# ajpowelsnl/mhm2_proxy

Hardware: AMD Instinct MI355X
Metric: k-mers/s (whole node), k=21 150bp reads (higher is better)
Workload: dtype u64

## Files before the change

mhm2_proxy_amd/csrc/kcount_kernels.hip:

```cpp
#include <hip/hip_runtime.h>
#include <type_traits>

#include <algorithm>

#include "kcount_launch.hpp"
#include "kmer_ops.hpp"

namespace mhm {

template <int NL>
constexpr int kTile() {
  return TILE_BASES[NL];
}
template <int NL>
constexpr int kEThreads() {
  return E_THREADS_NL[NL];
}
template <int NL>
constexpr int kPTile() {
  return P_TILE[NL];
}
template <int NL>
constexpr int kPThreads() {
  return P_THREADS[NL];
// ... 1357 lines not shown
    for (int i = threadIdx.x; i < SKETCH_FH; i += NT)
      if (fh[i]) atomicAdd(&fhist[i], fh[i]);
  for (int i = threadIdx.x; i < SKETCH_M; i += NT)
    if (reg[i]) {
      atomicMax(&hll[i], reg[i]);
      if (!(blockIdx.x & 1u)) atomicMax(&hll[SKETCH_M + 1 + i], reg[i]);
    }
  if (threadIdx.x == 0 && s_ext) atomicAdd(&hll[SKETCH_M], s_ext);
}

__global__ void k_init_fine(const unsigned long long *coarse_base, const unsigned long long *coarse_fcap, uint32_t n_coarse,
                            int fine_bits, unsigned long long *base, unsigned long long *cursor) {
  const uint64_t i = (uint64_t)blockIdx.x * blockDim.x + threadIdx.x;
  if (i >= ((uint64_t)n_coarse << fine_bits)) return;
  const uint64_t c = i >> fine_bits, d = i & ((1ull << fine_bits) - 1);
  const unsigned long long b = coarse_base[c] + d * coarse_fcap[c];
  base[i] = b;
  cursor[i] = b;
}

__global__ __launch_bounds__(256) void k_count_windows(ReadsView rv, int k, unsigned long long *out, unsigned int *err) {
  __shared__ unsigned long long s_acc[4];
  unsigned long long acc = 0;
  bool bad = false;
  const uint64_t stride = (uint64_t)gridDim.x * blockDim.x;
  for (uint64_t r0 = (uint64_t)blockIdx.x * blockDim.x + threadIdx.x; r0 < rv.n_reads; r0 += 4 * stride) {
    uint64_t a[4], b[4];
#pragma unroll
    for (int u = 0; u < 4; u++) {
      const uint64_t r = r0 + u * stride, rr = r < rv.n_reads ? r : rv.n_reads - 1;
      a[u] = rv.offs[rr];
      b[u] = rv.offs[rr + 1];
    }
#pragma unroll
    for (int u = 0; u < 4; u++) {
      if (r0 + u * stride >= rv.n_reads) break;
      bad |= b[u] < a[u] || b[u] - a[u] > 65535;
      const uint64_t L = b[u] - a[u];
      acc += (b[u] >= a[u] && L > (uint64_t)k + 1) ? L - k - 1 : 0;
    }
  }
  if (blockIdx.x == 0 && threadIdx.x == 0)
    bad |= rv.offs[0] != rv.obase + rv.head || rv.offs[rv.n_reads] - rv.obase != rv.n_bases;
  if (bad) atomicOr(err, 4u);
  acc = wave_sum_u64(acc);
  if ((threadIdx.x & 63) == 0) s_acc[threadIdx.x >> 6] = acc;
  __syncthreads();
  if (threadIdx.x == 0) {
    const unsigned long long t = s_acc[0] + s_acc[1] + s_acc[2] + s_acc[3];
    if (t) atomicAdd(out, t);
  }
}

__global__ __launch_bounds__(256) void k_expand_nibbles(const uint8_t *nib, uint8_t *arena, uint64_t b0, uint64_t n) {
  const uint64_t a0 = b0 & ~15ull, end = b0 + n;
  const uint64_t p0 = a0 + ((uint64_t)blockIdx.x * blockDim.x + threadIdx.x) * 16;
  if (p0 >= end) return;
  uint32_t w[4] = {0, 0, 0, 0};
#pragma unroll
  for (int i = 0; i < 16; i++) {
    const uint64_t p = p0 + i;
    if (p >= b0 && p < end) {
      const uint64_t j = p - b0;
      const uint32_t v = (nib[j >> 1] >> (4 * (uint32_t)(j & 1))) & 15u;
      w[i >> 2] |= ((v & 7u) | ((v >> 3) * 0xf8u)) << (8 * (i & 3));
    }
  }
  if (p0 >= b0 && p0 + 16 <= end) {
    *(uint4 *)(arena + p0) = make_uint4(w[0], w[1], w[2], w[3]);
    return;
  }
#pragma unroll
  for (int i = 0; i < 16; i++) {
    const uint64_t p = p0 + i;
    if (p >= b0 && p < end) arena[p] = (uint8_t)(w[i >> 2] >> (8 * (i & 3)));
  }
}

__global__ __launch_bounds__(256) void k_offs_from_deltas(const uint32_t *d, uint64_t *offs, uint64_t n, uint64_t b0) {
  for (uint64_t i = (uint64_t)blockIdx.x * 256 + threadIdx.x; i < n; i += (uint64_t)gridDim.x * 256) offs[i] = b0 + d[i];
}

__global__ __launch_bounds__(1024) void k_scan(const unsigned long long *in, unsigned long long *base,
                                               unsigned long long *cursor, uint32_t n) {
  __shared__ unsigned long long wsum[17];
  const int tid = threadIdx.x, lane = tid & 63, wid = tid >> 6;
  const uint32_t per = (n + 1023) / 1024;
  const uint32_t lo = min((uint32_t)tid * per, n), hi = min(lo + per, n);
  unsigned long long s = 0;
  for (uint32_t i = lo; i < hi; i++) s += (in[i] + 3) & ~3ull;
  unsigned long long x = s;
#pragma unroll
  for (int d = 1; d < 64; d <<= 1) {
    unsigned long long y = __shfl_up(x, d, 64);
    if (lane >= d) x += y;
  }
  if (lane == 63) wsum[wid] = x;
  __syncthreads();
  if (tid == 0) {
    unsigned long long acc = 0;
    for (int w = 0; w < 16; w++) {
      unsigned long long t = wsum[w];
      wsum[w] = acc;
      acc += t;
    }
  }
  __syncthreads();
  unsigned long long run = wsum[wid] + x - s;
  for (uint32_t i = lo; i < hi; i++) {
    base[i] = run;
    cursor[i] = run;
    run += (in[i] + 3) & ~3ull;
  }
}


template <int NL>
constexpr int count_rpt() {
  return NL == 1 ? 4 : 1;
}

template <int NL>
__device__ __forceinline__ uint32_t slot_hash(const uint64_t *key) {
  if (NL == 1) {
    const uint32_t x = (uint32_t)(key[0] >> 32) * 0x9E3779B1u + (uint32_t)key[0] * 0x85EBCA77u;
    return x ^ (x >> 15);
  }
  uint64_t h = key[0] * 0x9E3779B97F4A7C15ull;
#pragma unroll
  for (int w = 1; w < NL; w++) h = (h ^ (h >> 31) ^ key[w]) * 0xC2B2AE3D27D4EB4Full;
  h ^= h >> 29;
  return (uint32_t)(h >> 32);
}

__device__ __forceinline__ int cmp_group(uint32_t key, int kshl, uint32_t ng) {
  return (int)(__umul24((key << kshl) >> 16, ng) >> 16);
}

template <typename K>
struct CountLds {
  K *keys;
  uint32_t *cnt;
  uint32_t *ext;
  int cap;
};

typedef __attribute__((address_space(3))) unsigned int lds_u32_t;
__device__ __forceinline__ uint32_t lds_add_late(unsigned int *p, uint32_t v) {
  lds_u32_t *q = (lds_u32_t *)p;
  asm volatile("" : "+v"(q));
  return __hip_atomic_fetch_add(q, v, __ATOMIC_RELAXED, __HIP_MEMORY_SCOPE_WORKGROUP);
}

constexpr int C_PROBE = 64;
template <int NL>
constexpr int count_batch() {
  return NL == 2 ? 1 : 2;
}
constexpr int GS_SLOTS = 4;

template <int GS>
__device__ __forceinline__ void read_group(const uint64_t *last, int g, uint64_t (&v)[GS]) {
  const ulonglong2 *q = (const ulonglong2 *)(last + GS * g);
  const ulonglong2 a = q[0];
  v[0] = a.x, v[1] = a.y;
  if constexpr (GS == 4) {
    const ulonglong2 b = q[1];
    v[2] = b.x, v[3] = b.y;
  }
}
template <int GS>
__device__ __forceinline__ void read_group(const uint32_t *last, int g, uint32_t (&v)[GS]) {
  if constexpr (GS == 4) {
    const uint4 a = *(const uint4 *)(last + 4 * g);
    v[0] = a.x, v[1] = a.y, v[2] = a.z, v[3] = a.w;
  } else {
    const uint2 a = *(const uint2 *)(last + 2 * g);
    v[0] = a.x, v[1] = a.y;
  }
}

template <int NL, typename K>
__device__ __forceinline__ bool rest_equal(const CountLds<K> &t, int slot, const uint64_t *key) {
  bool eq = true;
#pragma unroll
  for (int w = 0; w < NL - 1; w++) eq &= (t.keys[w * t.cap + slot] == key[w]);
  return eq;
}

constexpr int G_FULL = -8, G_BUSY = -9;
template <int NL, int GS, typename K>
__device__ __forceinline__ int examine_group(const CountLds<K> &t, const uint64_t *key, int g, const K (&v)[GS]) {
  const K kl = (K)key[NL - 1];
  if constexpr (NL == 1) {
    int r = G_FULL;
#pragma unroll
    for (int i = GS - 1; i >= 0; i--) r = v[i] == (K)KEY_EMPTY ? -1 - i : r;
#pragma unroll
    for (int i = GS - 1; i >= 0; i--) r = v[i] == kl ? GS * g + i : r;
    return r;
  }
  if constexpr (NL >= 2) {
    int r = G_FULL;
#pragma unroll
    for (int i = GS - 1; i >= 0; i--) r = v[i] == (K)KEY_EMPTY ? -1 - i : r;
#pragma unroll
    for (int i = GS - 1; i >= 0; i--) r = v[i] == (K)KEY_BUSY ? G_BUSY : r;
#pragma unroll
    for (int i = GS - 1; i >= 0; i--) r = v[i] == kl ? GS * g + i : r;
    if (r < 0 || rest_equal<NL>(t, r, key)) return r;
  }
  int found = -1, empty = -1;
  bool busy = false;
#pragma unroll
  for (int i = 0; i < GS; i++) {
    if (found < 0 && v[i] == kl && (NL == 1 || rest_equal<NL>(t, GS * g + i, key))) found = i;
    if (v[i] == (K)KEY_EMPTY && empty < 0) empty = i;
    if (NL > 1 && v[i] == (K)KEY_BUSY) busy = true;
  }
  if (found >= 0) return GS * g + found;
  if (busy) return G_BUSY;
  return empty >= 0 ? -1 - empty : G_FULL;
}

template <int NL, int GS, typename K>
__device__ int lds_insert(const CountLds<K> &t, const uint64_t *key, int g, int r) {
  K *last = t.keys + (NL - 1) * t.cap;
  const int ng = t.cap / GS;
  const K kl = (K)key[NL - 1];
  int probed = 0;
  for (int iter = 0; iter < (1 << 20); iter++) {
    if (r >= 0) return r;
    if (r == G_FULL) {
      if (++probed == C_PROBE * 4 / GS) return -1;
      g = (g + 1 == ng) ? 0 : g + 1;
    } else if (r != G_BUSY) {
      const int sl = GS * g + (-1 - r);
      const K want = (NL == 1) ? kl : (K)KEY_BUSY;
      K old;
      if constexpr (sizeof(K) == 4)
        old = atomicCAS((unsigned int *)&last[sl], 0xffffffffu, (unsigned int)want);
      else
        old = atomicCAS((unsigned long long *)&last[sl], (unsigned long long)KEY_EMPTY, (unsigned long long)want);
      if (old == (K)KEY_EMPTY) {
        if (NL > 1) {
#pragma unroll
          for (int w = 0; w < NL - 1; w++) t.keys[w * t.cap + sl] = (K)key[w];
          __hip_atomic_store(&last[sl], kl, __ATOMIC_RELEASE, __HIP_MEMORY_SCOPE_WORKGROUP);
        }
        return sl;
      }
      if (NL == 1 && old == kl) return sl;
    }
    K v[GS];
    read_group<GS>(last, g, v);
    r = examine_group<NL, GS>(t, key, g, v);
  }
  return -2;
}

template <int NL, int GS, typename K>
__device__ __forceinline__ int claim_home(const CountLds<K> &t, const uint64_t *key, int g, int r) {
  K *last = t.keys + (NL - 1) * t.cap;
  const int sl = GS * g + (-1 - r);
  const K kl = (K)key[NL - 1];
  if constexpr (NL == 1) {
    K old;
    if constexpr (sizeof(K) == 4)
      old = atomicCAS((unsigned int *)&last[sl], 0xffffffffu, (unsigned int)kl);
    else
      old = atomicCAS((unsigned long long *)&last[sl], (unsigned long long)KEY_EMPTY, (unsigned long long)kl);
    return (old == (K)KEY_EMPTY || old == kl) ? sl : r;
  } else {
    const K old = atomicCAS((unsigned long long *)&last[sl], (unsigned long long)KEY_EMPTY, (unsigned long long)KEY_BUSY);
    if (old != (K)KEY_EMPTY) return r;
#pragma unroll
    for (int w = 0; w < NL - 1; w++) t.keys[w * t.cap + sl] = (K)key[w];
    __hip_atomic_store(&last[sl], kl, __ATOMIC_RELEASE, __HIP_MEMORY_SCOPE_WORKGROUP);
    return sl;
  }
}

template <typename K>
__device__ __forceinline__ uint32_t lds_add(const CountLds<K> &t, int slot, uint32_t e) {
  const uint32_t old = atomicAdd(&t.cnt[slot], 1u);
  const int l = (int)((e >> 3) & 7u), r = (int)(e & 7u);
  if (l < 4) atomicAdd(&t.ext[(l >> 1) * t.cap + slot], (l & 1) ? 0x10000u : 1u);
  if (r < 4) atomicAdd(&t.ext[(2 + (r >> 1)) * t.cap + slot], (r & 1) ? 0x10000u : 1u);
  return old;
}

template <typename K>
__device__ __forceinline__ void lds_add_nr(const CountLds<K> &t, int slot, uint32_t e, uint32_t *dummy) {
  const uint32_t l = (e >> 3) & 7u, r = e & 7u;
  uint32_t *lw = l < 4u ? &t.ext[(l >> 1) * t.cap + slot] : &t.cnt[slot];
  atomicAdd(lw, (l & 1u) ? 0x10000u : 1u);
  uint32_t *rw = r < 4u ? &t.ext[(2 + (r >> 1)) * t.cap + slot] : dummy;
  atomicAdd(rw, (r & 1u) ? 0x10000u : 1u);
}

template <typename K>
__device__ __forceinline__ uint32_t slot_count(const CountLds<K> &t, int slot, bool cold) {
  const uint32_t c = t.cnt[slot];
  if (!cold) return c;
  if (c >> 31) return c & 0x7fffffffu;
  const uint32_t e0 = t.ext[slot], e1 = t.ext[t.cap + slot];
  return c + (e0 & 0xffffu) + (e0 >> 16) + (e1 & 0xffffu) + (e1 >> 16);
}

__device__ __forceinline__ void ext_clamp(uint32_t *p, int half) {
  uint32_t cur = __hip_atomic_load(p, __ATOMIC_RELAXED, __HIP_MEMORY_SCOPE_WORKGROUP);
  for (int iter = 0; iter < 4096; iter++) {
    const uint32_t f = half ? (cur >> 16) : (cur & 0xffffu);
    if (f < 0xC000u) break;
    const uint32_t nw = half ? ((cur & 0xffffu) | 0x80000000u) : ((cur & 0xffff0000u) | 0x8000u);
    const uint32_t prev = atomicCAS(p, cur, nw);
    if (prev == cur) break;
    cur = prev;
  }
}

template <typename K>
__device__ __forceinline__ void lds_clamp(const CountLds<K> &t, int slot, uint32_t e) {
  const int l = (int)((e >> 3) & 7u), r = (int)(e & 7u);
  if (l < 4) ext_clamp(&t.ext[(l >> 1) * t.cap + slot], l & 1);
  if (r < 4) ext_clamp(&t.ext[(2 + (r >> 1)) * t.cap + slot], r & 1);
}

#ifndef MHMKC_STAMP
#define MHMKC_STAMP 0
#endif
#if MHMKC_STAMP
#define STAMP(var) const uint64_t var = __builtin_amdgcn_s_memtime()
#define STAMP_ADD(i, v) st_acc[i] += (v)
#else
#define STAMP(var)
#define STAMP_ADD(i, v)
#endif

__device__ __forceinline__ bool slot_survives(uint32_t c32, uint32_t e0, uint32_t e1, uint32_t e2, uint32_t e3,
                                              const CountParams &p, uint16_t &c16, char &L, char &R) {
  const uint32_t c = c32 > 65535u ? 65535u : c32;
  c16 = (uint16_t)c;
  const int thr = dyn_threshold(c, p.dyn_mult, p.dmin_thres);
  L = ext_choice(e0 & 0xffffu, e0 >> 16, e1 & 0xffffu, e1 >> 16, thr);
  R = ext_choice(e2 & 0xffffu, e2 >> 16, e3 & 0xffffu, e3 >> 16, thr);
  return !(L == 'X' && R == 'X');
}

template <int NL, bool CMP, typename K>
__device__ void ctg_apply(const CountLds<K> &t, const CountParams &p, uint32_t b, bool last_sweep, bool cold,
                          unsigned long long *s_range) {
  const int tid = threadIdx.x;
  if (tid == 0) {
    auto lower = [&](uint32_t v) {
      uint64_t lo = 0, hi = p.ctg_n;
      while (lo < hi) {
        const uint64_t mid = (lo + hi) >> 1;
        if (p.ctg_bucket[mid] < v)
          lo = mid + 1;
        else
          hi = mid;
      }
      return lo;
    };
    s_range[0] = lower(p.ctg_base + b);
    s_range[1] = lower(p.ctg_base + b + 1);
  }
  __syncthreads();
  const uint64_t q0 = s_range[0], q1 = s_range[1];
  constexpr int GS = GS_SLOTS;
  const int ng = t.cap / GS;
  const K *last = t.keys + (NL - 1) * t.cap;
  for (uint64_t q = q0 + tid; q < q1; q += C_THREADS) {
    if (p.ctg_done[q]) continue;
    uint64_t key[NL];
#pragma unroll
    for (int w = 0; w < NL; w++) key[w] = p.ctg_keys[w][q];
    const uint32_t st = p.ctg_state[q];
    const uint32_t c = st & 0xffffu, l = (st >> 16) & 7u, r = (st >> 19) & 7u;
    uint64_t tkey[NL];
#pragma unroll
    for (int w = 0; w < NL; w++) tkey[w] = key[w];
    if (RecKind<NL, CMP>::C32) {
      const int B = 2 * p.k, rb = B - p.coarse_bits - p.fine_bits;
      tkey[0] = (cmix(key[0] >> (64 - B), B) & ((1ull << rb) - 1)) << EXT_BITS;
    } else if (RecKind<NL, CMP>::M2) {
      uint64_t L, R;
      m2_mix(key, p.k, L, R);
      tkey[0] = (L & ((1ull << (p.k - p.coarse_bits - p.fine_bits)) - 1)) << EXT_BITS;
      tkey[NL - 1] = R;
    } else if (RecKind<NL, CMP>::MX) {
      uint64_t r[NL];
      mx_mix<NL>(key, r);
      tkey[0] = (r[0] & ((1ull << (64 - p.coarse_bits - p.fine_bits)) - 1)) << EXT_BITS;
#pragma unroll
      for (int w = 1; w < NL; w++) tkey[w] = r[w];
    }
    int g = RecKind<NL, CMP>::C32 ? cmp_group((uint32_t)tkey[0], 26 - (2 * p.k - p.coarse_bits - p.fine_bits), (uint32_t)ng)
            : RecKind<NL, CMP>::MW ? cmp_group((uint32_t)tkey[NL - 1], 16, (uint32_t)ng)
                                   : (int)__umulhi(slot_hash<NL>(tkey), (uint32_t)ng);
    int slot = -1;
    for (int pr = 0; pr < C_PROBE * 4 / GS; pr++) {
      K v[GS];
      read_group<GS>(last, g, v);
      const int e = examine_group<NL, GS>(t, tkey, g, v);
      if (e >= 0) {
        slot = e;
        break;
      }
      if (e != G_FULL) break;
      g = (g + 1 == ng) ? 0 : g + 1;
    }
    if (slot >= 0) {
      const uint32_t c32 = slot_count(t, slot, cold);
      const uint32_t rc = c32 > 65535u ? 65535u : c32;
      bool keep = false;
      if (rc >= 2) {
        const int thr = dyn_threshold(rc, p.dyn_mult, p.dmin_thres);
        const uint32_t e0 = t.ext[slot], e1 = t.ext[t.cap + slot], e2 = t.ext[2 * t.cap + slot],
                       e3 = t.ext[3 * t.cap + slot];
        const char L = ext_choice(e0 & 0xffffu, e0 >> 16, e1 & 0xffffu, e1 >> 16, thr);
        const char R = ext_choice(e2 & 0xffffu, e2 >> 16, e3 & 0xffffu, e3 >> 16, thr);
        keep = L != 'X' && L != 'F' && R != 'X' && R != 'F';
      }
      if (!keep) {
        const uint32_t h = c >= 0xC000u ? 0x8000u : c;
        uint32_t ew[4] = {0, 0, 0, 0};
        if (l < 4) ew[l >> 1] |= h << ((l & 1u) * 16);
        if (r < 4) ew[2 + (r >> 1)] |= h << ((r & 1u) * 16);
        t.cnt[slot] = cold ? 0x80000000u | c : c;
#pragma unroll
        for (int i = 0; i < 4; i++) t.ext[i * t.cap + slot] = ew[i];
      }
      p.ctg_done[q] = 1;
    } else if (last_sweep) {
      const int thr = dyn_threshold(c, p.dyn_mult, p.dmin_thres);
      uint32_t cl[4] = {0, 0, 0, 0}, cr[4] = {0, 0, 0, 0};
      if (l < 4) cl[l] = c;
      if (r < 4) cr[r] = c;
      const char L = ext_choice(cl[0], cl[1], cl[2], cl[3], thr), R = ext_choice(cr[0], cr[1], cr[2], cr[3], thr);
      atomicAdd(&p.stats[STAT_DISTINCT], 1ull);
      atomicAdd(&p.stats[STAT_COUNTSUM], (unsigned long long)c);
      if (c >= 2 && !(L == 'X' && R == 'X')) {
        const unsigned long long o = atomicAdd(p.out_cursor, 1ull);
        atomicAdd(&p.stats[STAT_NOUT], 1ull);
        if (o >= p.out_cap) {
          atomicOr(p.err, 16u);
          p.ctg_done[q] = 1;
          continue;
        }
// ... 65 lines not shown
  constexpr int MW = MC / (C_THREADS / 64);
  constexpr int WQ_THR = NL == 2 ? (MW < 64 ? MW : 64) : (MW / 2 < 64 ? MW / 2 : 64);
  const uint32_t wq_base = (uint32_t)__builtin_amdgcn_readfirstlane(threadIdx.x >> 6) * (uint32_t)MW;
  K *s_mkey = (K *)(smem + count_table_bytes(NL, RK::C32));
  uint32_t *s_me = (uint32_t *)(s_mkey + NL * MC);
  constexpr int SPT = (count_cap(NL, RK::C32) + C_THREADS - 1) / C_THREADS;
#ifndef MHMKC_KREG_NL
#define MHMKC_KREG_NL 3
#endif
#ifndef MHMKC_KJ
#define MHMKC_KJ 2
#endif
  constexpr bool KREG = NL <= MHMKC_KREG_NL;
  constexpr int KJ = KREG ? (MHMKC_KJ < SPT ? MHMKC_KJ : SPT) : 1;

#define tid (count_tid<NL>())
#define lane (count_tid<NL>() & 63)
#define wid (__builtin_amdgcn_readfirstlane(count_tid<NL>() >> 6))
  const uint64_t low_mask = (1ull << (EXT_BITS + p.hbits)) - 1;

  constexpr int R = count_rpt<NL>();
  constexpr uint32_t NONE = 0xffffffffu;
  constexpr uint32_t RND = (uint32_t)R * C_THREADS;
  constexpr uint32_t HOT = 0xC000u - 2u * (RND + (uint32_t)miss_cap(NL, RecKind<NL, CMP>::C32));
  static_assert(HOT > 0x8000u, "round too large for the extension-counter clamp");
  constexpr int C_BATCH = count_batch<NL>() < R ? count_batch<NL>() : R;
  static_assert(R % C_BATCH == 0, "batch must divide the records per round");
  constexpr int GS = GS_SLOTS;
  const int ng = t.cap / GS;
  const K *last = t.keys + (NL - 1) * t.cap;
  const int kshl = RK::C32 ? 26 - (2 * p.k - p.coarse_bits - p.fine_bits) : 16;

  uint64_t nk[R][NL];
  uint32_t nx[R];
  static_assert(!RK::C32 || R == 4, "compact rounds take one 16-byte load of 4 records per lane");
  struct Src {
    uint64_t off;
    uint32_t spl;
  };
  auto planes_of = [&](const Src &sr) -> PlaneSet {
    PlaneSet q = sr.spl ? p.spill : p.recs;
    const uint64_t o = sr.off;
    if (RK::C32) {
      q.w[0] = (uint64_t *)((uint32_t *)q.w[0] + o);
    } else if (RK::M2) {
      q.w[0] += 2 * o;
    } else {
#pragma unroll
      for (int w = 0; w < NL; w++) q.w[w] += o;
    }
    if (!PACKED) q.ext += o;
    return q;
  };
  auto prefetch = [&](const Src &sr, uint32_t cnt, uint32_t first, uint32_t nwv, uint32_t vt) {
    const PlaneSet src = planes_of(sr);
    const uint32_t dbase = first / RND * (uint32_t)(64 * R);
    if constexpr (RK::C32) {
      const uint32_t q = first + 4u * vt, qmax = (cnt - 1) & ~3u;
      const uint32_t qq = nwv == NONE ? (q < qmax ? q : qmax) : (dbase + 4u * (uint32_t)lane < nwv ? q : 0u);
      const u32x4 v = gload4((const uint32_t *)src.w[0] + qq);
      nk[0][0] = v.x;
      nk[1][0] = v.y;
      nk[2][0] = v.z;
      nk[3][0] = v.w;
#pragma unroll
      for (int j = 0; j < R; j++) nx[j] = 0;
      return;
    }
#pragma unroll
    for (int j = 0; j < R; j++) {
      const uint32_t i = first + vt + (uint32_t)j * C_THREADS;
      const uint32_t idx = nwv == NONE ? (i < cnt ? i : cnt - 1) : (dbase + (uint32_t)(64 * j + lane) < nwv ? i : 0u);
      if (RK::C32) {
        nk[j][0] = ((const uint32_t *)src.w[0])[idx];
      } else if (RK::M2) {
        const u32x4 v = gload4((const uint32_t *)src.w[0] + 4 * (uint64_t)idx);
        nk[j][0] = (uint64_t)v.x | ((uint64_t)v.y << 32);
        nk[j][NL - 1] = (uint64_t)v.z | ((uint64_t)v.w << 32);
      } else {
#pragma unroll
        for (int w = 0; w < NL; w++) nk[j][w] = src.w[w][idx];
      }
      nx[j] = PACKED ? 0u : (uint32_t)src.ext[idx];
    }
  };
  auto bucket_at = [&](uint64_t base, uint64_t end, Src &src, uint32_t &cnt) {
    cnt = (uint32_t)(end - base);
    src = Src{base, 0u};
  };
  auto bucket = [&](uint32_t bb, Src &src, uint32_t &cnt) { bucket_at(p.bucket_base[bb], p.bucket_end[bb], src, cnt); };

  auto defer_pos = [&]() -> uint32_t {
    (void)atomicAdd(&s_ovf, 1u);
    const uint32_t d = atomicAdd(&s_wdef[wid], 1u), rr = d / (uint32_t)(64 * R), rem = d % (uint32_t)(64 * R);
    return rr * RND + (RK::C32 ? (uint32_t)wid * 256u + rem : rem / 64u * C_THREADS + (uint32_t)wid * 64u + rem % 64u);
  };
  unsigned long long my_occ = 0, my_purged = 0, my_sum = 0, my_out = 0, my_sweeps = 0, my_maxb = 0;
  unsigned long long &s_missacc = s_u64[4];
#if MHMKC_STAMP
  uint64_t st_acc[6] = {0, 0, 0, 0, 0, 0};
  const uint64_t st_wg0 = __builtin_amdgcn_s_memtime();
#endif
  auto clear_table = [&]() {
    uint4 *ones = (uint4 *)(t.keys + (NL - 1) * t.cap);
    const int n_ones = t.cap * (int)sizeof(K) / 16;
    for (int i = tid; i < n_ones; i += C_THREADS) ones[i] = make_uint4(~0u, ~0u, ~0u, ~0u);
    uint4 *zeros = (uint4 *)t.cnt;
    const int n_zeros = t.cap * 20 / 16;
    for (int i = tid; i < n_zeros; i += C_THREADS) zeros[i] = make_uint4(0, 0, 0, 0);
  };
  auto reset_sweep = [&]() {
    if (tid == 0) {
      s_ovf = 0;
      s_err = 0;
      s_next = 2 * (C_THREADS / 64);
    }
    if (tid < C_THREADS / 64) s_wdef[tid] = 0;
  };
  if (tid == 0) {
    s_missacc = 0;
    s_u64[3] = 0;
  }
  clear_table();
  reset_sweep();
  __syncthreads();
  const Src spill{(uint64_t)blockIdx.x * SPILL_RECORDS, 1u};
  const bool has_spill = p.spill.w[0] != nullptr;
  uint32_t b = blockIdx.x;
  Src ps;
  uint32_t n;
  bucket(b, ps, n);
  if (n) prefetch(ps, n, 0, NONE, (uint32_t)tid);
  while (true) {
  my_maxb = my_maxb > n ? my_maxb : n;
  bool first_sweep = true;
  uint32_t nw = NONE, lim = n;
  bool dyn_sweep = false;
  Src pd = spill;
  uint32_t nb_next = 0;
  Src ps_next;
  const uint32_t b_next = b + gridDim.x;
  const uint32_t b_ext = b_next < p.n_buckets ? b_next : b;
  const uint64_t nx_base = p.bucket_base[b_ext], nx_end = p.bucket_end[b_ext];
  while (true) {
    if (!first_sweep && n) prefetch(ps, n, 0, nw, (uint32_t)tid);
    first_sweep = false;
    auto rounds = [&](auto cold_tag, auto dyn_tag) {
      constexpr bool COLD = decltype(cold_tag)::value;
      constexpr bool DYN = decltype(dyn_tag)::value;
      constexpr uint32_t NWV = C_THREADS / 64;
      int rnd = 0;
      uint32_t wq_n = 0;
      uint32_t cc = (uint32_t)wid, cn = (uint32_t)wid + NWV;
      auto slot_first = [&](uint32_t c) { return c / NWV * RND + c % NWV * (RK::C32 ? 256u : 64u); };
      for (uint32_t r0 = 0; DYN ? slot_first(cc) < n : r0 < lim; r0 += RND, rnd++) {
        STAMP(t_r0);
        uint64_t ck[R][NL];
        uint32_t ce[R];
        uint32_t ca = 0;
        if (DYN && lane == 0) ca = lds_add_late(&s_next, 1u);
        const uint32_t cr0 = DYN ? cc / NWV * RND : r0;
        const uint32_t vt = DYN ? cc % NWV * 64u + (uint32_t)lane : (uint32_t)tid;
        const uint32_t vfirst = nw == NONE ? cr0 + (RK::C32 ? 4u * vt : vt)
                                           : (uint32_t)rnd * (uint32_t)(64 * R) + (RK::C32 ? 4u * (uint32_t)lane : (uint32_t)lane);
        const uint32_t vend = nw == NONE ? n : nw;
        const uint32_t vrem = (vend > vfirst ? vend : vfirst) - vfirst;
        const uint32_t vstep = RK::C32 ? 1u : nw == NONE ? (uint32_t)C_THREADS : 64u;
#pragma unroll
        for (int j = 0; j < R; j++) {
          const bool valid = (uint32_t)j * vstep < vrem;
#pragma unroll
          for (int w = 0; w < NL; w++) ck[j][w] = nk[j][w];
          if (PACKED) {
            ce[j] = valid ? (uint32_t)(ck[j][RK::XW] & low_mask) : NONE;
            ck[j][RK::XW] &= ~low_mask;
          } else {
            ce[j] = valid ? nx[j] : NONE;
          }
        }
#if MHMKC_STAMP
#pragma unroll
        for (int j = 0; j < R; j++) asm volatile("" ::"v"(ck[j][0]), "v"(ce[j]));
#endif
        STAMP(t_r1);
        STAMP_ADD(1, t_r1 - t_r0);
        if (DYN)
          prefetch(ps, n, cn / NWV * RND, NONE, cn % NWV * 64u + (uint32_t)lane);
        else
          prefetch(ps, n, r0 + RND < lim ? r0 + RND : r0, nw, (uint32_t)tid);
        uint32_t old[R], defer = 0, okm = 0, missm = 0;
        int slot[R], g[R];
        if constexpr (RK::C32 && COLD) {
          K gv[R][GS];
          uint32_t res[R];
#pragma unroll
          for (int j = 0; j < R; j++) {
            g[j] = cmp_group((uint32_t)ck[j][0], kshl, (uint32_t)ng);
            read_group<GS>(last, g[j], gv[j]);
          }
#pragma unroll
          for (int j = 0; j < R; j++) slot[j] = examine_group<NL, GS>(t, ck[j], g[j], gv[j]);
#pragma unroll
          for (int j = 0; j < R; j++) {
            res[j] = 0u;
            if (ce[j] != NONE && slot[j] < 0 && slot[j] > G_FULL)
              res[j] = atomicCAS((unsigned int *)&last[GS * g[j] - 1 - slot[j]], 0xffffffffu, (uint32_t)ck[j][0]);
          }
#pragma unroll
          for (int j = 0; j < R; j++) {
            old[j] = 0;
            int r = slot[j];
            if (r < 0 && r > G_FULL && (res[j] == 0xffffffffu || res[j] == (uint32_t)ck[j][0])) r = GS * g[j] - 1 - r;
            if (ce[j] == NONE) {
              slot[j] = -3;
            } else if (r >= 0) {
              slot[j] = r;
              lds_add_nr(t, r, ce[j], &s_wave[wid]);
              okm |= 1u << j;
            } else {
              missm |= 1u << j;
            }
          }
        } else {
#pragma unroll
        for (int j0 = 0; j0 < R; j0 += C_BATCH) {
          K v[C_BATCH][GS];
#pragma unroll
          for (int j = j0; j < j0 + C_BATCH; j++) {
            g[j] = CMP ? cmp_group((uint32_t)ck[j][NL - 1], kshl, (uint32_t)ng)
                       : (int)__umulhi(slot_hash<NL>(ck[j]), (uint32_t)ng);
            read_group<GS>(last, g[j], v[j - j0]);
          }
#pragma unroll
          for (int j = j0; j < j0 + C_BATCH; j++) slot[j] = examine_group<NL, GS>(t, ck[j], g[j], v[j - j0]);
        }
#pragma unroll
        for (int j = 0; j < R; j++) {
          old[j] = 0;
          if (ce[j] == NONE) {
            slot[j] = -3;
            continue;
          }
          int r = slot[j];
          if (r < 0 && r > G_FULL) {
            const int sl = GS * g[j] + (-1 - r);
            r = claim_home<NL, GS>(t, ck[j], g[j], r);
            if (NL > 1 && r < 0) {
              const K v = __hip_atomic_load(&last[sl], __ATOMIC_ACQUIRE, __HIP_MEMORY_SCOPE_WORKGROUP);
              if (v == (K)ck[j][NL - 1] && rest_equal<NL>(t, sl, ck[j])) r = sl;
            }
            slot[j] = r;
          }
          if (r < 0) {
            missm |= 1u << j;
            slot[j] = r;
            continue;
          }
          if (COLD)
            lds_add_nr(t, r, ce[j], &s_wave[wid]);
          else
            old[j] = lds_add(t, r, ce[j]);
          okm |= 1u << j;
        }
        }
        {
#pragma unroll
          for (int j = 0; j < R; j++) {
            const bool mj = (missm >> j) & 1u;
            const uint64_t bal = __ballot(mj);
            const uint32_t tot = (uint32_t)__popcll(bal);
            if (wq_n + tot <= (uint32_t)MW) {
              if (mj) {
                const uint32_t q = wq_base + wq_n +
                                   __builtin_amdgcn_mbcnt_hi((uint32_t)(bal >> 32), __builtin_amdgcn_mbcnt_lo((uint32_t)bal, 0u));
#pragma unroll
                for (int w = 0; w < NL; w++) s_mkey[w * MC + q] = (K)ck[j][w];
                s_me[q] = ce[j];
                slot[j] = -3;
              }
              wq_n += tot;
            } else if (mj) {
              const int r = lds_insert<NL, GS>(t, ck[j], g[j], slot[j]);
              if (r == -1) defer |= 1u << j;
              if (r == -2) s_err = 1;
              slot[j] = r;
              if (r >= 0) {
                if (COLD)
                  lds_add_nr(t, r, ce[j], &s_wave[wid]);
                else
                  old[j] = lds_add(t, r, ce[j]);
                okm |= 1u << j;
              }
            }
          }
        }
#pragma unroll
        for (int j = 0; j < R; j++)
          if (!COLD && ((okm >> j) & 1u) && old[j] >= HOT) lds_clamp(t, slot[j], ce[j]);
        STAMP(t_r2);
        STAMP_ADD(2, t_r2 - t_r1);
        if (!COLD) __syncthreads();
        STAMP(t_r3);
        STAMP_ADD(3, t_r3 - t_r2);
        if (defer) {
#pragma unroll
          for (int j = 0; j < R; j++) {
            if ((defer >> j) & 1u) {
              if (DYN)
                store_record<NL, PACKED, CMP>(planes_of(pd), atomicAdd(&s_ovf, 1u), ck[j], ce[j]);
              else
                store_record<NL, PACKED, CMP>(planes_of(ps), defer_pos(), ck[j], ce[j]);
            }
          }
        }
        {
          const bool last_round = DYN ? slot_first(cn) >= n : r0 + RND >= lim;
          while (wq_n >= (uint32_t)WQ_THR || (last_round && wq_n > 0)) {
            const uint32_t take = wq_n < 64u ? wq_n : 64u;
            const uint32_t qb = wq_n - take;
            if ((uint32_t)lane < take) {
              const uint32_t q = wq_base + qb + (uint32_t)lane;
              uint64_t key[NL];
#pragma unroll
              for (int w = 0; w < NL; w++) key[w] = s_mkey[w * MC + q];
              const uint32_t e = s_me[q];
              const int g = CMP ? cmp_group((uint32_t)key[NL - 1], kshl, (uint32_t)ng)
                                : (int)__umulhi(slot_hash<NL>(key), (uint32_t)ng);
              K v[GS];
              read_group<GS>(last, g, v);
              const int r = lds_insert<NL, GS>(t, key, g, examine_group<NL, GS>(t, key, g, v));
              if (r >= 0) {
                if (COLD)
                  lds_add_nr(t, r, e, &s_wave[wid]);
                else if (lds_add(t, r, e) >= HOT)
                  lds_clamp(t, r, e);
              } else if (r == -1) {
                if (DYN)
                  store_record<NL, PACKED, CMP>(planes_of(pd), atomicAdd(&s_ovf, 1u), key, e);
                else
                  store_record<NL, PACKED, CMP>(planes_of(ps), defer_pos(), key, e);
              } else {
                s_err = 1;
              }
            }
            if (lane == 0) atomicAdd(&s_missacc, (unsigned long long)take);
            wq_n = qb;
          }
          if (DYN) {
            cc = cn;
            cn = __builtin_amdgcn_readfirstlane(ca);
          }
#if MHMKC_STAMP
          const uint64_t t_r4w = __builtin_amdgcn_s_memtime();
          STAMP_ADD(4, t_r4w - t_r3);
#endif
        }
      }
    };
    constexpr bool DYNS = NL <= DYN_SWEEP_MAX_NL;
    dyn_sweep = DYNS && has_spill && n < 0xC000u && (dyn_sweep || nw == NONE);
    const bool cold = DYNS ? dyn_sweep : n < 0xC000u;
    if constexpr (DYNS) {
      if (dyn_sweep)
        rounds(std::true_type{}, std::true_type{});
      else
        rounds(std::false_type{}, std::false_type{});
    } else {
      if (cold)
        rounds(std::true_type{}, std::false_type{});
      else
        rounds(std::false_type{}, std::false_type{});
    }
    STAMP(t_b0);
    __syncthreads();
    STAMP(t_f0);
    STAMP_ADD(3, t_f0 - t_b0);
    const bool last_sweep = s_ovf == 0;
    const uint32_t n_def = s_ovf;
    const bool err_sw = s_err != 0;
    uint32_t nw_def = 0, mx_def = 0;
    if (!last_sweep) {
      nw_def = s_wdef[wid];
#pragma unroll
      for (int w = 0; w < C_THREADS / 64; w++) mx_def = mx_def > s_wdef[w] ? mx_def : s_wdef[w];
      __builtin_amdgcn_fence(__ATOMIC_SEQ_CST, "agent");
    }
    if (p.ctg_n && !(p.coarse_skip && p.coarse_skip[b >> p.fine_bits])) ctg_apply<NL, CMP>(t, p, b, last_sweep, cold, s_red);
    {
      const bool nxt = last_sweep && b_next < p.n_buckets;
      if (nxt) bucket_at(nx_base, nx_end, ps_next, nb_next);
      const bool use_next = nxt && nb_next;
      prefetch(use_next ? ps_next : ps, use_next ? nb_next : (n ? n : 1u), 0, NONE, (uint32_t)tid);
    }

    uint16_t *flist = (uint16_t *)s_mkey;
    unsigned int *s_fin = (unsigned int *)(s_u64 + 3);
    uint32_t occ = 0;
    unsigned long long sum = 0;
    constexpr int QPT = (count_cap(NL, RK::C32) / 4 + C_THREADS - 1) / C_THREADS;
#pragma unroll
    for (int j = 0; j < QPT; j++) {
      const int qd = tid + j * C_THREADS;
      uint32_t c[4] = {0, 0, 0, 0};
      if (4 * qd < t.cap) {
        const uint4 c4 = *(const uint4 *)(t.cnt + 4 * qd);
        c[0] = c4.x, c[1] = c4.y, c[2] = c4.z, c[3] = c4.w;
        if (cold) {
          const uint4 a4 = *(const uint4 *)(t.ext + 4 * qd), b4 = *(const uint4 *)(t.ext + t.cap + 4 * qd);
          const uint32_t a[4] = {a4.x, a4.y, a4.z, a4.w}, bb[4] = {b4.x, b4.y, b4.z, b4.w};
#pragma unroll
          for (int i = 0; i < 4; i++)
            c[i] = (c[i] >> 31) ? c[i] & 0x7fffffffu
                                : c[i] + (a[i] & 0xffffu) + (a[i] >> 16) + (bb[i] & 0xffffu) + (bb[i] >> 16);
        }
      }
      uint64_t bal[4];
      uint32_t pre[4], tot = 0;
#pragma unroll
      for (int i = 0; i < 4; i++) {
        occ += c[i] != 0u;
        sum += c[i];
        bal[i] = __ballot(c[i] >= 2);
        pre[i] = tot;
        tot += (uint32_t)__popcll(bal[i]);
      }
      if (tot) {
        uint32_t fb = 0;
        if (lane == 0) fb = atomicAdd(&s_fin[0], tot);
        fb = __builtin_amdgcn_readfirstlane(fb);
#pragma unroll
        for (int i = 0; i < 4; i++)
          if (c[i] >= 2)
            flist[fb + pre[i] + __builtin_amdgcn_mbcnt_hi((uint32_t)(bal[i] >> 32),
                                                         __builtin_amdgcn_mbcnt_lo((uint32_t)bal[i], 0u))] =
                (uint16_t)(4 * qd + i);
      }
    }
    __syncthreads();
    const uint32_t n_list = s_fin[0];
    uint32_t surv_mask = 0, sp[SPT], row[SPT];
    const bool kfast = KREG && n_list <= (uint32_t)(KJ * C_THREADS);
    K kreg[KJ][NL];
#pragma unroll
    for (int j = 0; j < SPT; j++) {
      const uint32_t i = (uint32_t)tid + (uint32_t)j * C_THREADS;
      sp[j] = 0;
      row[j] = 0;
      bool sv = false;
      if (i < n_list) {
        const int slot = flist[i];
        sp[j] = (uint32_t)slot;
        uint16_t c16;
        char L, R_;
        const uint32_t cw = t.cnt[slot], e0 = t.ext[slot], e1 = t.ext[t.cap + slot], e2 = t.ext[2 * t.cap + slot],
                       e3 = t.ext[3 * t.cap + slot];
        if (KREG && j < KJ) {
#pragma unroll
          for (int w = 0; w < NL; w++) kreg[j < KJ ? j : 0][w] = t.keys[w * t.cap + slot];
        }
        const uint32_t c32 = !cold ? cw
                             : (cw >> 31) ? cw & 0x7fffffffu
                                          : cw + (e0 & 0xffffu) + (e0 >> 16) + (e1 & 0xffffu) + (e1 >> 16);
        sv = slot_survives(c32, e0, e1, e2, e3, p, c16, L, R_);
        row[j] = (uint32_t)c16 | (uint32_t)(uint8_t)L << 16 | (uint32_t)(uint8_t)R_ << 24;
      }
      const uint64_t bal = __ballot(sv);
      if (bal) {
        uint32_t sb = 0;
        if (lane == 0) sb = atomicAdd(&s_fin[1], (uint32_t)__popcll(bal));
        sb = __builtin_amdgcn_readfirstlane(sb);
        if (sv) {
          surv_mask |= 1u << j;
          sp[j] |= (sb + __builtin_amdgcn_mbcnt_hi((uint32_t)(bal >> 32), __builtin_amdgcn_mbcnt_lo((uint32_t)bal, 0u))) << 16;
        }
      }
    }
    const uint32_t mine = __popc(surv_mask);
    __syncthreads();
    unsigned long long gret = 0;
    uint32_t acc = 0;
    if (tid == 0) {
      acc = s_fin[1];
      if (acc) gret = atomicAdd(p.out_cursor, (unsigned long long)acc);
    }
    STAMP(t_c0);
    if (kfast) clear_table();
    STAMP(t_c1);
    reset_sweep();
    if (tid == 0) {
      unsigned long long gb = gret;
      if (acc && gb + acc > p.out_cap) {
        atomicOr(p.err, 16u);
        gb = ~0ull;
      }
      s_gbase = gb;
      my_out += acc;
      s_fin[0] = 0;
      s_fin[1] = 0;
    }
    __syncthreads();
    if (s_gbase == ~0ull) surv_mask = 0;
#pragma unroll
    for (int j = 0; j < SPT; j++) {
      if ((surv_mask >> j) & 1u) {
        const int slot = (int)(sp[j] & 0xffffu);
        auto kw_of = [&](int w) -> K { return (KREG && j < KJ && kfast) ? kreg[j < KJ ? j : 0][w] : t.keys[w * t.cap + slot]; };
        const unsigned long long g = s_gbase + (sp[j] >> 16);
        uint64_t *ok = p.out_keys + g * (uint64_t)p.nlo;
        if (RK::C32) {
          const int B = 2 * p.k, rb = B - p.coarse_bits - p.fine_bits;
          const uint64_t y = ((uint64_t)(p.bucket0 + b) << rb) | (kw_of(0) >> EXT_BITS);
          ok[0] = cunmix(y, B) << (64 - B);
        } else if (RK::M2) {
          const int rb = p.k - p.coarse_bits - p.fine_bits;
          const uint64_t L = ((uint64_t)(p.bucket0 + b) << rb) | (kw_of(0) >> EXT_BITS);
          uint64_t kw[2];
          m2_unmix(L, kw_of(1), p.k, kw);
          ok[0] = kw[0];
          ok[1] = kw[1];
        } else if (RK::MX) {
          const int rb = 64 - p.coarse_bits - p.fine_bits;
          uint64_t r[NL], kw[NL];
          r[0] = ((uint64_t)(p.bucket0 + b) << rb) | (kw_of(0) >> EXT_BITS);
#pragma unroll
          for (int w = 1; w < NL; w++) r[w] = kw_of(w);
          mx_unmix<NL>(r, kw);
#pragma unroll
          for (int w = 0; w < NL; w++) ok[w] = kw[w];
        } else {
#pragma unroll
          for (int w = 0; w < NL; w++) ok[w] = kw_of(w);
        }
        for (int w = NL; w < p.nlo; w++) ok[w] = 0;
        p.out_counts[g] = (uint16_t)row[j];
        p.out_left[g] = (char)(row[j] >> 16);
        p.out_right[g] = (char)(row[j] >> 24);
      }
    }
    my_occ += occ;
    my_purged += occ;
    my_purged -= mine;
    my_sum += sum;
    if (!kfast) {
      __syncthreads();
      clear_table();
      __syncthreads();
    }
    STAMP(t_f1);
    STAMP_ADD(0, t_c1 - t_c0);
    STAMP_ADD(5, t_f1 - t_f0 - (t_c1 - t_c0));
    if (err_sw && tid == 0) atomicAdd(&p.stats[STAT_N - 1], 1ull);
    if (last_sweep) break;
    n = n_def;
    lim = n;
    if (dyn_sweep) {
      const Src t_ = ps;
      ps = pd;
      pd = t_;
      nw = NONE;
    } else {
      nw = nw_def;
      lim = (mx_def + (uint32_t)(64 * R) - 1) / (uint32_t)(64 * R) * RND;
    }
    my_sweeps++;
    __builtin_amdgcn_fence(__ATOMIC_SEQ_CST, "agent");
  }
  if (b_next >= p.n_buckets) break;
  b = b_next;
  ps = ps_next;
  n = nb_next;
  pd = spill;
  dyn_sweep = false;
  }

#if MHMKC_STAMP
  if (lane == 0)
    for (int i = 0; i < 6; i++) atomicAdd(&p.stats[8 + i], (unsigned long long)st_acc[i]);
  if (tid == 0) {
    const uint64_t el = __builtin_amdgcn_s_memtime() - st_wg0;
    atomicAdd(&p.stats[14], (unsigned long long)el);
    atomicMax(&p.stats[15], (unsigned long long)el);
  }
#endif
  my_occ = wave_sum_u64(my_occ);
  my_purged = wave_sum_u64(my_purged);
  my_sum = wave_sum_u64(my_sum);
  if (tid == 0 && s_missacc) atomicAdd(&p.stats[STAT_MISSES], s_missacc);
  if (tid == 0) {
    s_red[0] = 0;
    s_red[1] = 0;
    s_red[2] = 0;
  }
  __syncthreads();
  if (lane == 0) {
    atomicAdd(&s_red[0], my_occ);
    atomicAdd(&s_red[1], my_purged);
    atomicAdd(&s_red[2], my_sum);
  }
  __syncthreads();
  if (tid == 0) {
    atomicAdd(&p.stats[STAT_DISTINCT], s_red[0]);
    atomicAdd(&p.stats[STAT_PURGED], s_red[1]);
    atomicAdd(&p.stats[STAT_COUNTSUM], s_red[2]);
    atomicAdd(&p.stats[STAT_NOUT], my_out);
    if (my_sweeps) atomicAdd(&p.stats[STAT_SWEEPS], my_sweeps);
    atomicMax(&p.stats[STAT_MAXBUCKET], my_maxb);
  }
}
#undef tid
#undef lane
#undef wid


#define MHM_DISPATCH(nl, packed, FN, ARGS)   \
  switch ((nl) * 2 + ((packed) ? 1 : 0)) {   \
    case 2: return FN<1, false> ARGS;        \
    case 3: return FN<1, true> ARGS;         \
    case 4: return FN<2, false> ARGS;        \
    case 5: return FN<2, true> ARGS;         \
    case 6: return FN<3, false> ARGS;        \
    case 7: return FN<3, true> ARGS;         \
    case 8: return FN<4, false> ARGS;        \
    case 9: return FN<4, true> ARGS;         \
    default: return hipErrorInvalidValue;    \
  }
#define MHM_DISPATCH_MIXED(nl, FN, ARGS)                                                                \
  ((nl) == 1 ? FN<1, true, true> ARGS : (nl) == 2 ? FN<2, true, true> ARGS : (nl) == 3 ? FN<3, true, true> ARGS \
             : (nl) == 4 ? FN<4, true, true> ARGS : hipErrorInvalidValue)

template <typename K>
static hipError_t allow_lds(K kernel, size_t lds) {
  if (lds <= 65536) return hipSuccess;
  return hipFuncSetAttribute((const void *)kernel, hipFuncAttributeMaxDynamicSharedMemorySize, (int)lds);
}

template <int NL, bool PK, bool CMP = false>
static hipError_t do_extract_hist(const ExtractParams &p, hipStream_t s) {
  const size_t lds = tile_lds_bytes<NL>() + (size_t)p.n_bins * 4;
  hipError_t e = allow_lds(k_extract_hist<NL, PK, CMP>, lds);
  if (e != hipSuccess) return e;
  k_extract_hist<NL, PK, CMP><<<dim3(p.n_tiles), dim3(kEThreads<NL>()), lds, s>>>(p);
  return hipGetLastError();
}

template <int NL, bool PK, bool CMP = false>
static hipError_t do_extract_scatter(const ExtractParams &p, hipStream_t s) {
  const size_t lds = staged_cnt_bytes(p.n_bins) +
                     std::max(tile_lds_bytes<NL>(),
                              staged_area_bytes(NL, kECap<NL>(), PK, RecKind<NL, CMP>::C32 ? SF_C40 : SF_WORDS));
  if (p.n_bins <= (uint32_t)kEThreads<NL>()) {
    hipError_t e = allow_lds(k_extract_scatter<NL, PK, CMP, 1>, lds);
    if (e != hipSuccess) return e;
    k_extract_scatter<NL, PK, CMP, 1><<<dim3(p.n_tiles), dim3(kEThreads<NL>()), lds, s>>>(p);
    return hipGetLastError();
  }
  hipError_t e = allow_lds(k_extract_scatter<NL, PK, CMP>, lds);
// ... 281 lines not shown
```

Baseline: 110.3 billion.

## Use contiguous dynamic work slots, LUT-based LDS ext adds, and early-exit finalize loops

Dynamic work distribution in the counting rounds now hands each wave a contiguous slot of records rather than interleaved chunks. The code can also split the final tail slots into smaller sub-slots to balance the end of the work, although the default divisor of 1 leaves that off. The LDS extension-count update uses a shift-based lookup that computes the plane index and increment without branches, and assumes cnt and ext are laid out contiguously at cap stride. The finalize loop makes the list length wave-uniform and exits early once a wave's index passes the survivor list, which skips empty iterations. Together these aim to cut tail imbalance, ALU/branch overhead per k-mer, and wasted finalize passes, at the cost of relying on an implicit table-layout assumption.

```diff
diff --git a/mhm2_proxy_amd/csrc/kcount_kernels.hip b/mhm2_proxy_amd/csrc/kcount_kernels.hip
--- a/mhm2_proxy_amd/csrc/kcount_kernels.hip
+++ b/mhm2_proxy_amd/csrc/kcount_kernels.hip
@@ -1533,6 +1533,18 @@
   return __hip_atomic_fetch_add(q, v, __ATOMIC_RELAXED, __HIP_MEMORY_SCOPE_WORKGROUP);
 }
 
+#ifndef MHMKC_TAIL_DIV
+#define MHMKC_TAIL_DIV 1
+#endif
+#ifndef MHMKC_TAIL_SLOTS
+#define MHMKC_TAIL_SLOTS 4
+#endif
+#ifndef MHMKC_TAIL_DIV2
+#define MHMKC_TAIL_DIV2 1
+#endif
+#ifndef MHMKC_TAIL_SLOTS2
+#define MHMKC_TAIL_SLOTS2 4
+#endif
 constexpr int C_PROBE = 64;
 template <int NL>
 constexpr int count_batch() {
@@ -1671,13 +1683,23 @@
   return old;
 }
 
+#ifndef MHMKC_ADDLUT
+#define MHMKC_ADDLUT 1
+#endif
 template <typename K>
 __device__ __forceinline__ void lds_add_nr(const CountLds<K> &t, int slot, uint32_t e, uint32_t *dummy) {
+#if MHMKC_ADDLUT
+  const uint32_t pl = (0x2211u >> ((e >> 1) & 0x1cu)) & 3u, r = e & 7u;
+  atomicAdd(&t.cnt[pl * (uint32_t)t.cap + (uint32_t)slot], 1u << ((e & 8u) << 1));
+  if (r < 4u) atomicAdd(&t.cnt[(3u + (r >> 1)) * (uint32_t)t.cap + (uint32_t)slot], 1u << ((e & 1u) << 4));
+  (void)dummy;
+#else
   const uint32_t l = (e >> 3) & 7u, r = e & 7u;
   uint32_t *lw = l < 4u ? &t.ext[(l >> 1) * t.cap + slot] : &t.cnt[slot];
   atomicAdd(lw, (l & 1u) ? 0x10000u : 1u);
   uint32_t *rw = r < 4u ? &t.ext[(2 + (r >> 1)) * t.cap + slot] : dummy;
   atomicAdd(rw, (r & 1u) ? 0x10000u : 1u);
+#endif
 }
 
 template <typename K>
@@ -2049,20 +2071,35 @@
       int rnd = 0;
       uint32_t wq_n = 0;
       uint32_t cc = (uint32_t)wid, cn = (uint32_t)wid + NWV;
-      auto slot_first = [&](uint32_t c) { return c / NWV * RND + c % NWV * (RK::C32 ? 256u : 64u); };
+      constexpr uint32_t SLOT = 64u * (uint32_t)R;
+      static_assert(RND == NWV * SLOT, "a round is one wave slot per wave");
+      constexpr bool CONTIG = RK::C32 || R == 1;
+      constexpr uint32_t TAIL_DIV = !CONTIG ? 1 : NL == 1 ? MHMKC_TAIL_DIV : MHMKC_TAIL_DIV2;
+      constexpr uint32_t TAIL_SLOTS = NL == 1 ? MHMKC_TAIL_SLOTS : MHMKC_TAIL_SLOTS2;
+      constexpr uint32_t SUB = SLOT / TAIL_DIV;
+      static_assert(TAIL_DIV >= 1 && SUB * TAIL_DIV == SLOT && SUB % (uint32_t)R == 0, "sub-slots are whole lanes' records");
+      const uint32_t n_slots = (n + SLOT - 1) / SLOT;
+      const uint32_t t0 = n_slots > 2 * NWV + TAIL_SLOTS ? n_slots - TAIL_SLOTS : 2 * NWV;
+      auto slot_first = [&](uint32_t c) -> uint32_t {
+        if constexpr (!CONTIG) return c / NWV * RND + c % NWV * 64u;
+        if constexpr (TAIL_DIV == 1) return c * SLOT;
+        return c < t0 ? c * SLOT : t0 * SLOT + (c - t0) * SUB;
+      };
+      auto slot_size = [&](uint32_t c) -> uint32_t { return TAIL_DIV == 1 || c < t0 ? SLOT : SUB; };
       for (uint32_t r0 = 0; DYN ? slot_first(cc) < n : r0 < lim; r0 += RND, rnd++) {
         STAMP(t_r0);
         uint64_t ck[R][NL];
         uint32_t ce[R];
         uint32_t ca = 0;
         if (DYN && lane == 0) ca = lds_add_late(&s_next, 1u);
-        const uint32_t cr0 = DYN ? cc / NWV * RND : r0;
-        const uint32_t vt = DYN ? cc % NWV * 64u + (uint32_t)lane : (uint32_t)tid;
-        const uint32_t vfirst = nw == NONE ? cr0 + (RK::C32 ? 4u * vt : vt)
-                                           : (uint32_t)rnd * (uint32_t)(64 * R) + (RK::C32 ? 4u * (uint32_t)lane : (uint32_t)lane);
-        const uint32_t vend = nw == NONE ? n : nw;
+        const uint32_t cfirst = DYN ? slot_first(cc) : 0u;
+        const uint32_t vfirst = DYN          ? cfirst + (RK::C32 ? 4u * (uint32_t)lane : (uint32_t)lane)
+                                : nw == NONE ? r0 + (RK::C32 ? 4u * (uint32_t)tid : (uint32_t)tid)
+                                             : (uint32_t)rnd * (uint32_t)(64 * R) + (RK::C32 ? 4u * (uint32_t)lane : (uint32_t)lane);
+        const uint32_t cend = DYN && CONTIG ? cfirst + slot_size(cc) : n;
+        const uint32_t vend = DYN ? (cend < n ? cend : n) : nw == NONE ? n : nw;
         const uint32_t vrem = (vend > vfirst ? vend : vfirst) - vfirst;
-        const uint32_t vstep = RK::C32 ? 1u : nw == NONE ? (uint32_t)C_THREADS : 64u;
+        const uint32_t vstep = RK::C32 ? 1u : (DYN || nw == NONE) ? (uint32_t)C_THREADS : 64u;
 #pragma unroll
         for (int j = 0; j < R; j++) {
           const bool valid = (uint32_t)j * vstep < vrem;
@@ -2082,7 +2119,7 @@
         STAMP(t_r1);
         STAMP_ADD(1, t_r1 - t_r0);
         if (DYN)
-          prefetch(ps, n, cn / NWV * RND, NONE, cn % NWV * 64u + (uint32_t)lane);
+          prefetch(ps, n, CONTIG ? slot_first(cn) : cn / NWV * RND, NONE, (CONTIG ? 0u : cn % NWV * 64u) + (uint32_t)lane);
         else
           prefetch(ps, n, r0 + RND < lim ? r0 + RND : r0, nw, (uint32_t)tid);
         uint32_t old[R], defer = 0, okm = 0, missm = 0;
@@ -2334,15 +2371,20 @@
       }
     }
     __syncthreads();
-    const uint32_t n_list = s_fin[0];
+#ifndef MHMKC_FINX
+#define MHMKC_FINX 1
+#endif
+    const uint32_t n_list = MHMKC_FINX ? (uint32_t)__builtin_amdgcn_readfirstlane(s_fin[0]) : s_fin[0];
+    const uint32_t fin_w0 = (uint32_t)wid * 64u;
     uint32_t surv_mask = 0, sp[SPT], row[SPT];
+#pragma unroll
+    for (int j = 0; j < SPT; j++) sp[j] = 0, row[j] = 0;
     const bool kfast = KREG && n_list <= (uint32_t)(KJ * C_THREADS);
     K kreg[KJ][NL];
 #pragma unroll
     for (int j = 0; j < SPT; j++) {
+      if (MHMKC_FINX && fin_w0 + (uint32_t)j * C_THREADS >= n_list) break;
       const uint32_t i = (uint32_t)tid + (uint32_t)j * C_THREADS;
-      sp[j] = 0;
-      row[j] = 0;
       bool sv = false;
       if (i < n_list) {
         const int slot = flist[i];
@@ -2399,6 +2441,7 @@
     if (s_gbase == ~0ull) surv_mask = 0;
 #pragma unroll
     for (int j = 0; j < SPT; j++) {
+      if (MHMKC_FINX && fin_w0 + (uint32_t)j * C_THREADS >= n_list) break;
       if ((surv_mask >> j) & 1u) {
         const int slot = (int)(sp[j] & 0xffffu);
         auto kw_of = [&](int w) -> K { return (KREG && j < KJ && kfast) ? kreg[j < KJ ? j : 0][w] : t.keys[w * t.cap + slot]; };
```

After: 115.8 billion, median of 6. 1.05x the previous value.
